# anneouyang/OuterSPACE

Measured on AMD Instinct MI355X. Metric: spgemm_output_nnz_per_s, higher is better.
Workload: dtype f64

## Files before the change

outerspace_amd/csrc/osp_kernels.h:

```cpp
#pragma once
#include <type_traits>
#include "osp_prims.h"

namespace osp {

template <class T> struct TileCap;
#ifndef OSP_TILE_CAP_F32
#define OSP_TILE_CAP_F32 1792
#endif
template <> struct TileCap<float> { static constexpr int value = OSP_TILE_CAP_F32; };
#ifndef OSP_TILE_CAP_F64
#define OSP_TILE_CAP_F64 1536
#endif
template <> struct TileCap<double> { static constexpr int value = OSP_TILE_CAP_F64; };
constexpr int kMergeThreads = 256;
constexpr int kTileMaxRows = kMergeThreads - 1;
constexpr int kMulThreads = 256;
#ifndef OSP_MUL_PER_WAVE
#define OSP_MUL_PER_WAVE 2048
#endif
constexpr int kMulPerWave = OSP_MUL_PER_WAVE;
constexpr int kMulPerBlock = kMulPerWave * (kMulThreads / kWave);
#ifndef OSP_MUL_BATCH_MAX
#define OSP_MUL_BATCH_MAX 4096
// ... 1005 lines not shown
                d.rcnt = vrun_end[rb - 1] - d.rbeg;
            }
        }
    }
    desc[pos] = d;
}
__global__ void chain_rows_kernel(const uint32_t *heavy_rows, uint32_t nlong, const uint32_t *tile_rows0, uint32_t ntiles0,
                                  const uint64_t *vbase, const uint32_t *tile_rows1, uint32_t ntiles1, uint32_t *j0,
                                  uint32_t *tb, uint32_t *cntm1) {
    const uint32_t h = blockIdx.x * blockDim.x + threadIdx.x;
    if (h > nlong) return;
    if (h == nlong) { tb[h] = ntiles1; return; }
    j0[h] = (uint32_t)lower_bound_dev(tile_rows0, 0, (uint64_t)ntiles0, heavy_rows[h]);
    const uint32_t b = (uint32_t)lower_bound_dev(tile_rows1, 0, (uint64_t)ntiles1, vbase[h]);
    const uint32_t e = (uint32_t)lower_bound_dev(tile_rows1, 0, (uint64_t)ntiles1, vbase[h + 1]);
    tb[h] = b;
    cntm1[h] = e - b - 1;
}
__global__ void chain_finish_kernel(const uint32_t *heavy_rows, uint32_t nlong, const uint64_t *vbase, const int64_t *vptr,
                                    const uint64_t *out_end, uint64_t r_end, int64_t *c_rowptr) {
    const uint32_t h = blockIdx.x * blockDim.x + threadIdx.x;
    if (h < nlong) c_rowptr[heavy_rows[h]] = vptr[vbase[h]];
    if (h == 0) c_rowptr[r_end] = (int64_t)*out_end;
}

#ifdef OSP_CHECK_DESC
__device__ unsigned long long osp_desc_bad[16];
#define OSP_DESC_CHECK(t_, d_) do { if ((t_) < ntiles) { const TileDesc g_ = desc[(t_)]; \
    if (g_.s != (d_).s || g_.n != (d_).n || g_.ra != (d_).ra || g_.nr != (d_).nr || g_.lvl != (d_).lvl) { \
        if (atomicAdd(&osp_desc_bad[0], 1ull) == 0) { osp_desc_bad[1] = (t_); osp_desc_bad[2] = tid; osp_desc_bad[3] = (d_).s; osp_desc_bad[4] = g_.s; \
            osp_desc_bad[5] = (d_).n; osp_desc_bad[6] = g_.n; osp_desc_bad[7] = (d_).lvl; osp_desc_bad[8] = blockIdx.x; osp_desc_bad[9] = NT; } \
        (d_) = g_; } } } while (0)
__device__ unsigned long long *osp_crumbs;
#define OSP_CRUMB(ph_, a_, b_, c_) do { if (tid == 0 && osp_crumbs) { volatile unsigned long long *p_ = osp_crumbs + (size_t)(blockIdx.x & 4095u) * 8u; \
    p_[1] = t; p_[2] = d.s; p_[3] = d.n; p_[4] = (a_); p_[5] = (b_); p_[6] = (c_); p_[7] = d.ra; \
    p_[0] = (unsigned long long)(ph_) | ((unsigned long long)NT << 8) | ((unsigned long long)ABL << 32); __threadfence_system(); } } while (0)
#else
#define OSP_DESC_CHECK(t_, d_)
#define OSP_CRUMB(ph_, a_, b_, c_)
#endif

#ifdef OSP_MERGE_PROF
__device__ unsigned long long osp_merge_prof[16];
#define OSP_PROF_DECL __shared__ unsigned long long prof_acc[12]; if (tid < 12) prof_acc[tid] = 0; __syncthreads(); unsigned long long prof_t = clock64();
#define OSP_PROF_MARK(k) do { if (tid == 0) { const unsigned long long now_ = clock64(); prof_acc[k] += now_ - prof_t; prof_t = now_; } } while (0)
#define OSP_PROF_FLUSH do { if (tid == 0) for (int k_ = 0; k_ < 12; k_++) atomicAdd(&osp_merge_prof[k_], prof_acc[k_]); } while (0)
#else
#define OSP_PROF_DECL
#define OSP_PROF_MARK(k)
#define OSP_PROF_FLUSH
#endif

constexpr int kMergeMaxWgs = 5;
template <class T, int NT, int CAP, int MAXWG = kMergeMaxWgs, int ABL = 0>
constexpr int merge_wgs_per_cu() {
    const int wgs = (160 * 1024) / (int)(sizeof(MergeSmem<T, NT, CAP>) + ((ABL & 64) ? CAP * sizeof(T) : 0) + 64);
    return wgs > MAXWG ? MAXWG : wgs;
}
template <class T, int NT, int CAP, int MAXWG = kMergeMaxWgs, int ABL = 0>
constexpr int merge_waves_per_simd() {
    const int w = (merge_wgs_per_cu<T, NT, CAP, MAXWG, ABL>() * NT + 255) / 256;
    return w > 8 ? 8 : (w < 1 ? 1 : w);
}
template <class T, int NT, int ABL = 0, int CAP = TileCap<T>::value, int MAXWG = kMergeMaxWgs, bool RA = (OSP_RANK_ATOMIC != 0), bool GA = false>
__global__ __launch_bounds__(NT, (merge_waves_per_simd<T, NT, CAP, MAXWG, ABL>())) void merge_tiles_kernel(
    const TileDesc *__restrict__ desc, uint32_t ntiles, const MergeLevels<T> lvl, int colbits, uint64_t *tile_status,
    uint32_t *ticket, const uint64_t *__restrict__ out_base_p, uint32_t *__restrict__ c_col, T *__restrict__ c_val,
    uint64_t *__restrict__ out_end_p, const ChunkTable<T> ct = ChunkTable<T>{}, uint32_t nshards = 1, uint32_t *abort_word = nullptr,
    const GatherArgs<T> ga = GatherArgs<T>{}) {
    __shared__ MergeSmem<T, NT, CAP> sm;
    __shared__ TileDesc s_dnext;
    __shared__ uint32_t s_tnext;
    constexpr bool ROWWISE = (ABL & 64) != 0;
    __shared__ T rwval[ROWWISE ? CAP : 1];
    constexpr int kTileCap = CAP;
    constexpr int NW = NT / kWave;
    constexpr int LPT = (kTileCap + NT - 1) / NT;
    constexpr int ITERS = (kTileCap / NW + kWave - 1) / kWave;
    constexpr int IPT = LPT;
    constexpr int DPT = (kDigits + NT - 1) / NT;
    static_assert(kTileMaxRows + 1 <= NT, "row offsets are fetched one per thread");
    unsigned tid = threadIdx.x, lane = lane_id(), w = tid >> 6;
    uint32_t shard = 0;
    if constexpr (GA) { if (tid < (uint32_t)kTileCap / 32u) sm.gbits[tid] = 0; }
    if (tid == 0) {
        if (nshards > 1) shard = atomicAdd(&ticket[nshards * kTicketStride], 1u) % nshards;
        const uint32_t t0 = (ABL & 4) ? blockIdx.x : take_ticket(ticket, nshards, shard, ntiles);
        s_tnext = t0;
        if (t0 < ntiles) s_dnext = desc[t0];
    }
    __syncthreads();
#ifndef OSP_TEST_NO_LATE_GUARD
    if (s_tnext >= ntiles) return;
#endif
    const uint64_t out_base = (ABL & 32) ? 0ull : *out_base_p;
    const uint32_t colmask = colbits < 32 ? ((1u << colbits) - 1u) : 0xffffffffu;
    uint32_t t = s_tnext;
    TileDesc d = s_dnext;
    OSP_CRUMB(5, ntiles, d.lvl, d.nr);
    uint64_t ro = 0;
    PartWords<T> lrec[LPT];
    constexpr uint32_t kSpan = (uint32_t)kTileCap / NW;
    static_assert(!GA || (kTileCap % (NW * kWave) == 0 && (int)kSpan == LPT * kWave), "gathered tiles: a wave's span is LPT wave-loads");
    uint32_t ix0 = GA ? w * kSpan + lane : tid;
    constexpr uint32_t ixs = GA ? (uint32_t)kWave : (uint32_t)NT;
    auto request = [&](const TileDesc &dd, bool ok) {
        bool fetch = ok && dd.n <= (uint32_t)kTileCap;
        ro = 0;
#ifndef OSP_TEST_NO_LATE_GUARD
        const uint32_t lv_i = dd.lvl & 1u;
#else
        const uint32_t lv_i = dd.lvl;
#endif
        const Part<T> *__restrict__ stage = lvl.stage[lv_i];
        if (fetch && tid <= dd.nr) ro = lvl.row_off[lv_i][dd.ra + tid];
        if (ROWWISE && dd.lvl == 0) fetch = false;
        if constexpr (GA) {
            if (fetch && dd.rcnt != 0) {
                typedef uint32_t u32x2 __attribute__((ext_vector_type(2)));
                const RunDesc<T> *__restrict__ gruns = dd.lvl ? ga.runs : ga.runs0;
                const u32x2 ds2 = *reinterpret_cast<const u32x2 *>(&gruns[tid < dd.rcnt ? dd.rbeg + tid : dd.rbeg]);
                const u32x2 ds3 = *reinterpret_cast<const u32x2 *>(&gruns[tid + NT < dd.rcnt ? dd.rbeg + tid + NT : dd.rbeg]);
                lrec[0].w[0] = ds2.x;
                lrec[0].w[1] = ds2.y;
                lrec[1].w[0] = ds3.x;
                lrec[1].w[1] = ds3.y;
                return;
            }
        }
#pragma unroll
        for (int q = 0; q < LPT; q++) {
            const uint32_t i = ix0 + q * ixs;
            const Part<T> *src = (fetch && i < dd.n) ? &stage[dd.s + i] : reinterpret_cast<const Part<T> *>(desc);
            lrec[q] = load_part_words(src);
        }
    };
    request(d, t < ntiles);
    __syncthreads();
    OSP_PROF_DECL
    while (t < ntiles) {
        if constexpr (GA) { asm volatile("" : "+v"(tid)); lane = tid & 63u; w = tid >> 6; ix0 = w * kSpan + lane; }
        OSP_DESC_CHECK(t, d);
        OSP_CRUMB(1, ntiles, d.lvl, d.nr);
        const uint64_t ra = d.ra, s = d.s, base = lvl.base[d.lvl];
        const uint32_t nr = d.nr, n = d.n;
        int64_t *__restrict__ c_rowptr = lvl.c_rowptr[d.lvl];
        const bool long_row = n > (uint32_t)kTileCap;
        uint32_t tn_reg = ntiles;
        if (long_row) {
            if (w == 0) {
                const uint64_t total = lvl.heavy_nnz[d.lvl][ra];
                const uint64_t excl = (ABL & 2) ? (uint64_t)t * kTileCap : lookback_prefix(tile_status, t, total, abort_word);
                if (lane == 0) {
                    tn_reg = (ABL & 4) ? t + gridDim.x : take_ticket(ticket, nshards, shard, ntiles);
                    c_rowptr[ra] = (int64_t)(out_base + excl);
                    if (t + 1 == ntiles) *out_end_p = out_base + excl + total;
                    s_tnext = tn_reg;
                    if (tn_reg < ntiles) s_dnext = desc[tn_reg];
                }
            }
            __syncthreads();
            t = s_tnext;
            d = s_dnext;
            request(d, t < ntiles);
            __syncthreads();
            continue;
        }
        int rowbits = 0;
        while ((1u << rowbits) < nr) rowbits++;
        const bool relkey = d.kbits != 0;
        const uint32_t cbase = d.cbase;
        const int keybits = relkey ? (int)d.kbits : colbits + rowbits;
        const int nbits = (n && !(ABL & 1)) ? keybits : 0;
        constexpr uint32_t HS = MergeSmem<T, NT, CAP>::kHashWords;
        typedef MergeSmem<T, NT, CAP> Smem;
        static_assert(!OSP_HASH_IN_CNT || offsetof(Smem, cnt) + sizeof(sm.cnt) == offsetof(Smem, pos0) + 4u * HS,
                      "hash table: from pos0 through the digit counters without a gap");
        uint32_t *htab = sm.htab();
        constexpr bool INPLACE = (ABL & 32) != 0;
        const bool early = nbits > 0 && keybits < 32 && !(ABL & 2) && !(ABL & 8) && !INPLACE;
        const bool gath = GA && d.rcnt != 0;
        uint32_t kq[LPT];
        T vq[LPT];
        uint32_t rq[(LPT + 1) / 2];
        constexpr bool kRunInPad = GA && Smem::kWide;
        constexpr bool kKeepPos = GA && Smem::kWide;
        uint32_t bpos[LPT];
        constexpr uint32_t GW = GA ? (uint32_t)kTileCap : 0u;
        constexpr uint32_t HSG = HS - GW;
        uint32_t *gsrc = htab, *htab_g = htab + GW;
        if constexpr (GA) {
            if (gath) {
                static_assert(HS > 2 * GW, "gathered tiles: the run table leaves a hash table of more than two words per entry... of half the entries");
                const uint32_t R = d.rcnt, tile0 = (uint32_t)(s + base);
                const RunDesc<T> *__restrict__ gruns = d.lvl ? ga.runs : ga.runs0;
                for (uint32_t x = tid; x < R; x += NT) {
                    uint32_t dst = lrec[0].w[0], src = lrec[0].w[1];
                    if (x == tid + NT) { dst = lrec[1].w[0]; src = lrec[1].w[1]; }
                    else if (x != tid) { const RunDesc<T> rd = gruns[d.rbeg + x]; dst = rd.dst; src = rd.src; }
                    const uint32_t st = dst - tile0;
                    gsrc[x] = src - st;
                    atomicOr(&sm.gbits[st >> 5], 1u << (st & 31u));
                }
                if (early) {
                    typedef uint32_t u32x4 __attribute__((ext_vector_type(4)));
                    static_assert((offsetof(Smem, pos0) + 4u * GW) % 16 == 0, "gathered tiles: the hash table starts 16-byte aligned");
                    constexpr uint32_t nvec = HSG / 4, tail = HSG % 4;
                    u32x4 *hv = reinterpret_cast<u32x4 *>(htab_g);
                    const u32x4 ones = {0xffffffffu, 0xffffffffu, 0xffffffffu, 0xffffffffu};
                    for (uint32_t i = tid; i < nvec; i += NT) hv[i] = ones;
                    if (tid < tail) htab_g[nvec * 4 + tid] = 0xffffffffu;
                    if (tid == 0) sm.hcount = 0;
                }
            }
        }
        if (!gath && early) {
            if constexpr (ABL & 256) {
                for (uint32_t i = tid; i < HS; i += NT) htab[i] = 0xffffffffu;
            } else {
                static_assert((kTileCap * 4) % 8 == 0, "hash table: 16-byte groups behind an 8-byte aligned start (odd words at both ends singly)");
                typedef uint32_t u32x4 __attribute__((ext_vector_type(4)));
                constexpr uint32_t lead = ((kTileCap * 4) % 16) / 4;
                constexpr uint32_t nvec = (HS - lead) / 4, tail = (HS - lead) % 4;
                u32x4 *hv = reinterpret_cast<u32x4 *>(htab + lead);
                const u32x4 ones = {0xffffffffu, 0xffffffffu, 0xffffffffu, 0xffffffffu};
                for (uint32_t i = tid; i < nvec; i += NT) hv[i] = ones;
                if (tid < lead) htab[tid] = 0xffffffffu;
                if (tid < tail) htab[lead + nvec * 4 + tid] = 0xffffffffu;
            }
            if (tid == 0) sm.hcount = 0;
        }
        if (tid <= nr) sm.rowo[tid] = (uint32_t)(ro - base - s);
        __syncthreads();
        OSP_PROF_MARK(0);
        uint32_t fresh = 0;
        const bool rw_tile = ROWWISE && d.lvl == 0;
        if constexpr (GA) {
            if (gath) {
                uint32_t cnt0 = 0;
                {
                    const uint32_t nwords = w * (kSpan / 32u);
                    static_assert((NW - 1) * (kSpan / 32u) <= (uint32_t)kWave, "gathered tiles: the bits before a wave's span, one word per lane");
                    cnt0 = wave_reduce_sum<uint32_t>(lane < nwords ? (uint32_t)__popc(sm.gbits[lane]) : 0u);
                    cnt0 = (uint32_t)__builtin_amdgcn_readfirstlane((int)cnt0);
                }
#pragma unroll
                for (int q = 0; q < (LPT + 1) / 2; q++) rq[q] = 0;
#pragma unroll
                for (int q = 0; q < LPT; q++) {
                    const uint32_t i = ix0 + q * ixs;
                    const uint32_t wi = w * (kSpan / 32u) + 2u * (uint32_t)q;
                    const uint32_t mlo = sm.gbits[wi], mhi = sm.gbits[wi + 1];
                    const uint32_t below = __builtin_amdgcn_mbcnt_hi(mhi, __builtin_amdgcn_mbcnt_lo(mlo, 0u));
                    const uint32_t own = ((lane < 32 ? mlo >> lane : mhi >> (lane - 32)) & 1u);
                    const uint32_t r = cnt0 + below + own - 1u;
                    cnt0 += (uint32_t)__popc(mlo) + (uint32_t)__popc(mhi);
                    bpos[q] = i < n ? gsrc[r] + i : 0u;
                    rq[q >> 1] |= (i < n ? r : 0u) << (16 * (q & 1));
                }
                uint32_t bc[LPT];
#pragma unroll
                for (int q = 0; q < LPT; q++) bc[q] = ga.b_colidx[bpos[q]];
#pragma unroll
                for (int q = 0; q < LPT; q++) {
                    const uint32_t i = ix0 + q * ixs;
                    if (relkey) {
                        kq[q] = bc[q] - cbase;
                    } else {
                        uint32_t lo = 0, hi = nr;
                        while (hi - lo > 1) { const uint32_t mid = (lo + hi) >> 1; if (sm.rowo[mid] <= i) lo = mid; else hi = mid; }
                        kq[q] = (colbits < 32 ? (lo << colbits) : 0u) | bc[q];
                    }
                    if (i < n) sm.key0[i] = kq[q];
                }
                OSP_PROF_MARK(11);
                if (early) {
                    uint32_t hq[LPT], oq[LPT];
#pragma unroll
                    for (int q = 0; q < LPT; q++) {
                        hq[q] = (uint32_t)(((uint64_t)(kq[q] * 2654435761u) * HSG) >> 32);
                        oq[q] = kq[q];
                        if (ix0 + q * ixs < n) oq[q] = atomicCAS(&htab_g[hq[q]], 0xffffffffu, kq[q]);
                    }
#pragma unroll
                    for (int q = 0; q < LPT; q++) {
                        if (ix0 + q * ixs < n) {
                            uint32_t old = oq[q], h = hq[q];
                            while (old != 0xffffffffu && old != kq[q]) {
                                h = (h + 1 == HSG) ? 0u : h + 1;
                                old = atomicCAS(&htab_g[h], 0xffffffffu, kq[q]);
                            }
                            fresh += old == 0xffffffffu;
                        }
                    }
                }
            }
        }
        if (gath) {
        } else if (rw_tile) {
            if constexpr (ROWWISE) {
                constexpr uint32_t kRwGroup = 16, kRwSteps = 4, kRwUnroll = 4;
                const uint32_t c0 = ct.rowfirst[ra], c1 = ct.rowfirst[ra + nr];
                for (uint32_t cb = c0 + w * kRwGroup; cb < c1; cb += NW * kRwGroup) {
                    const uint32_t c = cb + lane;
                    const bool cv = lane < kRwGroup && c < c1;
                    const uint64_t o0 = cv ? ct.off[c] : 0ull, o1 = cv ? ct.off[c + 1] : 0ull;
                    const uint32_t st = cv ? (uint32_t)(o0 - base - s) : n;
                    const uint32_t en = cv ? (uint32_t)(o1 - base - s) : n;
                    const uint32_t bsv = cv ? ct.bs[c] : 0u;
                    const T av = cv ? ct.a_vals[ct.perm[c]] : T(0);
                    uint32_t lrow = 0;
                    {
                        uint32_t lo = 0, hi = nr;
                        while (hi - lo > 1) { const uint32_t mid = (lo + hi) >> 1; if (sm.rowo[mid] <= st) lo = mid; else hi = mid; }
                        lrow = colbits < 32 ? (lo << colbits) : 0u;
                    }
                    const uint32_t nvalid = min(kRwGroup, c1 - cb);
                    const uint32_t gbeg = wave_bcast(st, 0u), gend = wave_bcast(en, nvalid - 1);
                    for (uint32_t ib0 = gbeg; ib0 < gend; ib0 += kRwUnroll * kWave) {
                        uint32_t bcol[kRwUnroll], crow[kRwUnroll];
                        T bval[kRwUnroll], cav[kRwUnroll];
#pragma unroll
                        for (uint32_t u = 0; u < kRwUnroll; u++) {
                            const uint32_t i = ib0 + u * kWave + lane;
                            uint32_t lo = 0, hi = kRwGroup;
#pragma unroll
                            for (uint32_t step = 0; step < kRwSteps; step++) {
                                const uint32_t mid = (lo + hi) >> 1;
                                const uint32_t sv = (uint32_t)__shfl((int)st, (int)mid);
                                if (sv <= i) lo = mid; else hi = mid;
                            }
                            const uint32_t cst = (uint32_t)__shfl((int)st, (int)lo);
                            const uint32_t cbs = (uint32_t)__shfl((int)bsv, (int)lo);
                            crow[u] = (uint32_t)__shfl((int)lrow, (int)lo);
                            cav[u] = __shfl(av, (int)lo);
                            const uint32_t b = i < gend ? cbs + (i - cst) : 0u;
                            bcol[u] = ct.b_colidx[b];
                            bval[u] = ct.b_vals[b];
                        }
#pragma unroll
                        for (uint32_t u = 0; u < kRwUnroll; u++) {
                            const uint32_t i = ib0 + u * kWave + lane;
                            if (i < gend) {
                                const uint32_t key = crow[u] | bcol[u];
                                sm.key0[i] = key;
                                rwval[i] = cav[u] * bval[u];
                                if (early) {
                                    uint32_t h = (uint32_t)(((uint64_t)(key * 2654435761u) * HS) >> 32);
                                    uint32_t old = atomicCAS(&htab[h], 0xffffffffu, key);
                                    while (old != 0xffffffffu && old != key) {
                                        h = (h + 1 == HS) ? 0u : h + 1;
                                        old = atomicCAS(&htab[h], 0xffffffffu, key);
                                    }
                                    fresh += old == 0xffffffffu;
                                }
                            }
                        }
                    }
                }
            }
        } else {
#pragma unroll
            for (int q = 0; q < LPT; q++) {
                const uint32_t i = ix0 + q * ixs;
                kq[q] = 0;
                if (i < n) {
                    if (relkey) {
                        kq[q] = lrec[q].col() - cbase;
                    } else {
                        uint32_t lo = 0, hi = nr;
                        while (hi - lo > 1) { const uint32_t mid = (lo + hi) >> 1; if (sm.rowo[mid] <= i) lo = mid; else hi = mid; }
                        kq[q] = (colbits < 32 ? (lo << colbits) : 0u) | lrec[q].col();
                    }
                    sm.key0[i] = kq[q];
                }
            }
            if (early) {
                uint32_t hq[LPT], oq[LPT];
#pragma unroll
                for (int q = 0; q < LPT; q++) {
                    hq[q] = (uint32_t)(((uint64_t)(kq[q] * 2654435761u) * HS) >> 32);
                    oq[q] = kq[q];
                    if (ix0 + q * ixs < n) oq[q] = atomicCAS(&htab[hq[q]], 0xffffffffu, kq[q]);
                }
#pragma unroll
                for (int q = 0; q < LPT; q++) {
                    if (ix0 + q * ixs < n) {
                        uint32_t old = oq[q], h = hq[q];
                        while (old != 0xffffffffu && old != kq[q]) {
                            h = (h + 1 == HS) ? 0u : h + 1;
                            old = atomicCAS(&htab[h], 0xffffffffu, kq[q]);
                        }
                        fresh += old == 0xffffffffu;
                    }
                }
            }
        }
        if (early) {
            const uint32_t wsum = wave_incl_scan(fresh);
            if (lane == kWave - 1 && wsum) atomicAdd(&sm.hcount, wsum);
        }
        const uint32_t per = (n + NW - 1) / NW;
        const uint32_t wbeg = min(w * per, n), wend = min(wbeg + per, n);
        int cur = 0;
        __syncthreads();
        if constexpr (GA) {
            if (gath) {
                if (tid < (uint32_t)kTileCap / 32u) sm.gbits[tid] = 0;
                if constexpr (kRunInPad) {
#pragma unroll
                    for (int q = 0; q < LPT; q++) {
                        const uint32_t i = ix0 + q * ixs;
                        if (i < n) sm.pad[i] = (uint16_t)(rq[q >> 1] >> (16 * (q & 1)));
                    }
                }
            }
        }
        OSP_PROF_MARK(1);
        if (early && tid == 0) lookback_publish(tile_status, t, sm.hcount);
        OSP_PROF_MARK(2);
        const int npass = (nbits + kDigitBits - 1) / kDigitBits;
        const int pbits = npass ? (nbits + npass - 1) / npass : 0;
        const uint32_t dmask = (1u << pbits) - 1u;
        const int ndig = 1 << pbits;
        for (int pass = 0, shift = 0; pass < npass; pass++, shift += pbits) {
            uint32_t *ksrc = sm.key(cur), *kdst = sm.key(cur ^ 1);
            uint16_t *psrc = sm.pos(cur), *pdst = sm.pos(cur ^ 1);
            if constexpr (ABL & 128) {
                for (int dd = lane; dd < ndig; dd += kWave) sm.cnt[w][dd] = 0;
            } else {
                uint64_t *c64 = reinterpret_cast<uint64_t *>(sm.cnt[w]);
                for (int dd = lane; dd < (ndig + 3) / 4; dd += kWave) c64[dd] = 0ull;
            }
            uint32_t kreg[ITERS], rreg[ITERS];
            auto rank_span = [&](auto bits_tag) {
                constexpr int BITS = decltype(bits_tag)::value;
#pragma unroll
                for (int it = 0; it < ITERS; it++) {
                    const uint32_t i = wbeg + it * kWave + lane;
                    const bool valid = i < wend;
                    kreg[it] = valid ? ksrc[i] : 0u;
                    const unsigned dg = (kreg[it] >> shift) & dmask;
                    unsigned rk, cntd;
                    wave_match_digit<BITS>(dg, valid, rk, cntd);
                    rreg[it] = 0;
                    if (valid) {
                        const uint32_t c = sm.cnt[w][dg];
                        rreg[it] = c + rk;
                        if (rk == 0) sm.cnt[w][dg] = (uint16_t)(c + cntd);
                    }
                }
            };
            if constexpr (RA) {
            {
                uint32_t(*cnt32)[kDigits / 2] = reinterpret_cast<uint32_t(*)[kDigits / 2]>(sm.cnt);
#pragma unroll
                for (int it = 0; it < ITERS; it++) {
                    const uint32_t i = wbeg + it * kWave + lane;
                    const bool valid = i < wend;
                    kreg[it] = valid ? ksrc[i] : 0u;
                    const unsigned dg = (kreg[it] >> shift) & dmask;
                    const unsigned half = 16u * (dg & 1u);
                    rreg[it] = 0;
                    if (valid) rreg[it] = (atomicAdd(&cnt32[w][dg >> 1], 1u << half) >> half) & 0xffffu;
                }
                (void)rank_span;
            }
            } else {
            if (pbits > kDigitBits - 1) rank_span(std::integral_constant<int, kDigitBits>{});
            else rank_span(std::integral_constant<int, kDigitBits - 1>{});
            }
            __syncthreads();
            OSP_PROF_MARK(3);
            if constexpr ((ABL & 128) != 0 || DPT != 4) {
                const int dpt = (ndig + NT - 1) / NT;
                uint32_t c[DPT][NW], ssum = 0;
#pragma unroll
                for (int q = 0; q < DPT; q++) {
                    const int dg = tid * dpt + q;
                    const bool on = q < dpt && dg < ndig;
#pragma unroll
                    for (int ww = 0; ww < NW; ww++) { c[q][ww] = on ? sm.cnt[ww][dg] : 0u; ssum += c[q][ww]; }
                }
                uint32_t total;
                uint32_t ex = block_excl_scan<uint32_t, NT, false>(ssum, sm.scratch, &total)  ;
#pragma unroll
                for (int q = 0; q < DPT; q++) {
                    const int dg = tid * dpt + q;
                    if (q < dpt && dg < ndig) {
#pragma unroll
                        for (int ww = 0; ww < NW; ww++) { sm.cnt[ww][dg] = (uint16_t)ex; ex += c[q][ww]; }
                    }
                }
            } else {
                const bool on = (int)tid * 4 < ndig;
                uint64_t pk[NW];
                uint32_t ssum = 0;
#pragma unroll
                for (int ww = 0; ww < NW; ww++) {
                    pk[ww] = on ? reinterpret_cast<const uint64_t *>(sm.cnt[ww])[tid] : 0ull;
                    ssum += (uint32_t)(pk[ww] & 0xffffu) + (uint32_t)((pk[ww] >> 16) & 0xffffu) + (uint32_t)((pk[ww] >> 32) & 0xffffu) +
                            (uint32_t)(pk[ww] >> 48);
                }
                uint32_t total;
                uint32_t ex = block_excl_scan<uint32_t, NT, false>(ssum, sm.scratch, &total)  ;
                if (on) {
                    uint32_t o[4][NW];
#pragma unroll
                    for (int q = 0; q < 4; q++) {
#pragma unroll
                        for (int ww = 0; ww < NW; ww++) { o[q][ww] = ex; ex += (uint32_t)(pk[ww] >> (16 * q)) & 0xffffu; }
                    }
#pragma unroll
                    for (int ww = 0; ww < NW; ww++)
                        reinterpret_cast<uint64_t *>(sm.cnt[ww])[tid] = (uint64_t)(o[0][ww] & 0xffffu) | ((uint64_t)(o[1][ww] & 0xffffu) << 16) |
                                                                        ((uint64_t)(o[2][ww] & 0xffffu) << 32) | ((uint64_t)(o[3][ww] & 0xffffu) << 48);
                }
            }
            __syncthreads();
            OSP_PROF_MARK(4);
#pragma unroll
            for (int it = 0; it < ITERS; it++) {
                const uint32_t i = wbeg + it * kWave + lane;
                if (i < wend) {
                    const uint32_t k = kreg[it];
                    const uint32_t dst = (uint32_t)sm.cnt[w][(k >> shift) & dmask] + rreg[it];
                    kdst[dst] = k;
                    pdst[dst] = pass == 0 ? (uint16_t)i : psrc[i];
                }
            }
            cur ^= 1;
            __syncthreads();
            OSP_PROF_MARK(5);
        }
        uint32_t *skey = sm.key(cur);
        uint16_t *spos = sm.pos(cur);
        T *sval = rw_tile ? rwval : sm.vals(cur);
        if (npass == 0) {
            for (uint32_t i = tid; i < n; i += NT) spos[i] = (uint16_t)i;
        }
        OSP_CRUMB(2, npass, cur, nbits);
        if (!rw_tile && !gath) {
            const Part<T> *__restrict__ stg = lvl.stage[d.lvl];
#pragma unroll
            for (int q = 0; q < LPT; q++) {
                const uint32_t i = ix0 + q * ixs;
                vq[q] = load_part_words(i < n ? &stg[s + i] : reinterpret_cast<const Part<T> *>(desc)).val();
            }
        }
        if constexpr (GA) {
            if (gath) {
                const uint32_t tile0 = (uint32_t)(s + base);
                const RunDesc<T> *__restrict__ gruns = d.lvl ? ga.runs : ga.runs0;
                T bv[LPT];
                if constexpr (kKeepPos) {
                    T av[LPT];
#pragma unroll
                    for (int q = 0; q < LPT; q++) {
                        const uint32_t i = ix0 + q * ixs;
                        bv[q] = ga.b_vals[bpos[q]];
                        av[q] = gruns[d.rbeg + (i < n ? (uint32_t)sm.pad[i] : 0u)].av;
                    }
#pragma unroll
                    for (int q = 0; q < LPT; q++) vq[q] = av[q] * bv[q];
                    (void)tile0;
                } else {
                RunDesc<T> rdq[LPT];
#pragma unroll
                for (int q = 0; q < LPT; q++) {
                    const uint32_t i = ix0 + q * ixs;
                    uint32_t r;
                    if constexpr (kRunInPad) r = i < n ? (uint32_t)sm.pad[i] : 0u;
                    else r = (rq[q >> 1] >> (16 * (q & 1))) & 0xffffu;
                    rdq[q] = gruns[d.rbeg + r];
                }
#pragma unroll
                for (int q = 0; q < LPT; q++) {
                    const uint32_t i = ix0 + q * ixs;
                    bv[q] = ga.b_vals[i < n ? rdq[q].src - (rdq[q].dst - tile0) + i : 0u];
                }
#pragma unroll
                for (int q = 0; q < LPT; q++) vq[q] = rdq[q].av * bv[q];
                }
            }
        }
        if (npass == 0) __syncthreads();
        const uint32_t ib = tid * IPT;
        uint32_t heads = 0, hmask = 0;
#pragma unroll
        for (int q = 0; q < IPT; q++) {
            const uint32_t i = ib + q;
            if (i < n) {
                const bool h = (i == 0) || (skey[i] != skey[i - 1]);
                hmask |= (h ? 1u : 0u) << q;
                heads += h;
            }
        }
        if constexpr (kRunInPad) {
            if (gath) __syncthreads();
        }
        if (!rw_tile) {
#pragma unroll
            for (int q = 0; q < LPT; q++) {
                const uint32_t i = ix0 + q * ixs;
                if (i < n) sval[i] = vq[q];
            }
        }
        if (tid == 0) sm.nlongrun = 0;
        uint32_t total;
        uint32_t ex = block_excl_scan<uint32_t, NT, false>(heads, sm.scratch, &total);
        OSP_PROF_MARK(6);
        if (w == 0) {
            const uint64_t excl = INPLACE   ? 0ull
                                 : (ABL & 2) ? (uint64_t)t * kTileCap
                                 : early     ? lookback_prefix<false>(tile_status, t, total, abort_word)
                                             : lookback_prefix<true>(tile_status, t, total, abort_word);
            if (lane == 0) {
                sm.excl = excl;
                tn_reg = (ABL & 4) ? t + gridDim.x : take_ticket(ticket, nshards, shard, ntiles);
            }
        }
        OSP_PROF_MARK(7);
        const uint32_t oslot0 = ex;
#pragma unroll
        for (int q = 0; q < IPT; q++) {
            const uint32_t i = ib + q;
            if (i < n) {
                sm.rank[i] = (uint16_t)ex;
                ex += (hmask >> q) & 1u;
            }
        }
        if (tid == 0) sm.rank[n] = (uint16_t)total;
        static_assert(IPT <= kRunShort, "the part of a run inside one thread's entries is never longer than a head's own share");
        T acc[IPT];
        uint32_t ocol[IPT], lmask = 0, tmask = 0;
        {
            T v[IPT];
#pragma unroll
            for (int q = 0; q < IPT; q++) {
                const uint32_t i = ib + q;
                v[q] = i < n ? sval[spos[i]] : T(0);
            }
            T cur = T(0);
#pragma unroll
            for (int q = 0; q < IPT; q++) {
                const uint32_t i = ib + q;
                const bool hd = (hmask >> q) & 1u;
                cur = hd ? v[q] : cur + v[q];
                const bool nexthd = q + 1 < IPT ? ((hmask >> (q + 1)) & 1u) != 0 : true;
                const bool tail = i < n && (i + 1 >= n || nexthd) && (hmask & ((2u << q) - 1u)) != 0;
                acc[q] = cur;
                ocol[q] = 0;
                tmask |= (tail ? 1u : 0u) << q;
            }
        }
        if (tmask) {
            const int qt = 31 - __builtin_clz(tmask);
            const uint32_t it = ib + (uint32_t)qt;
            if (qt == IPT - 1 && it + 1 < n) {
                const uint32_t ih = ib + (uint32_t)(31 - __builtin_clz(hmask));
                const uint32_t k = skey[it];
                T a = acc[IPT - 1];
                const uint32_t ulim = min(n, ih + (uint32_t)kRunShort);
                uint32_t u = it + 1;
                for (; u < ulim && skey[u] == k; u++) a += sval[spos[u]];
                if (u == ulim && u < n && skey[u] == k) {
                    const uint32_t idx = atomicAdd(&sm.nlongrun, 1u);
                    sm.long_sum()[idx] = a;
                    sm.long_pos()[idx] = (uint16_t)u;
                    lmask |= 1u << (IPT - 1);
                    a = index_as_value<T>(idx);
                }
                acc[IPT - 1] = a;
            }
#pragma unroll
            for (int q = 0; q < IPT; q++) {
                if ((tmask >> q) & 1u) {
                    const uint32_t k = skey[ib + q];
                    ocol[q] = relkey ? k + cbase : (k & colmask);
                }
            }
        }
        if (tid == 0) s_tnext = tn_reg;
        __syncthreads();
        if (const uint32_t nlr = sm.nlongrun) {
            T *lsum = sm.long_sum();
            const uint16_t *lpos = sm.long_pos();
            for (uint32_t r = w; r < nlr; r += NW) {
                const uint32_t u1 = lpos[r], k = skey[u1];
                T a = lsum[r];
                for (uint32_t u0 = u1;; u0 += kWave) {
                    const uint32_t u = u0 + lane;
                    const bool in = u < n && skey[u] == k;
                    const T v = in ? sval[spos[u]] : T(0);
                    const uint64_t m = __ballot(in);
                    const uint32_t c = m == ~0ull ? (uint32_t)kWave : (uint32_t)__builtin_ctzll(~m);
                    for (uint32_t x = 0; x < c; x++) a += wave_bcast(v, x);
                    if (c < (uint32_t)kWave) break;
                }
                if (lane == 0) lsum[r] = a;
            }
            __syncthreads();
        }
        OSP_PROF_MARK(8);
#pragma unroll
        for (int q = 0; q < IPT; q++) {
            if ((tmask >> q) & 1u) {
                const uint32_t slot = oslot0 + (uint32_t)__popc(hmask & ((2u << q) - 1u)) - 1u;
                skey[slot] = ocol[q];
                sval[slot] = ((lmask >> q) & 1u) ? sm.long_sum()[value_as_index<T>(acc[q])] : acc[q];
            }
        }
        if (tid == 0 && tn_reg < ntiles) s_dnext = desc[tn_reg];
        __syncthreads();
        OSP_PROF_MARK(9);
        const uint32_t tn = s_tnext;
        const TileDesc dn = s_dnext;
        OSP_CRUMB(3, total, tn, dn.s);
        request(dn, tn < ntiles);
        if constexpr (INPLACE) {
            Part<T> *outp = const_cast<Part<T> *>(lvl.stage[d.lvl]) + s;
            for (uint32_t o = tid; o < total; o += NT) outp[o] = Part<T>{skey[o], sval[o]};
            if (tid == 0) const_cast<uint32_t *>(lvl.heavy_nnz[d.lvl])[ra] = total;
        } else {
            const uint64_t obase = out_base + sm.excl;
            for (uint32_t o = tid; o < total; o += NT) {
                __builtin_nontemporal_store(skey[o], &c_col[obase + o]);
                __builtin_nontemporal_store(sval[o], &c_val[obase + o]);
            }
            if (tid < nr) c_rowptr[ra + tid] = (int64_t)(obase + sm.rank[sm.rowo[tid]]);
            if (t + 1 == ntiles && tid == 0) *out_end_p = obase + total;
        }
        OSP_CRUMB(4, total, tn, 0);
        t = tn;
        d = dn;
        __syncthreads();
        OSP_PROF_MARK(10);
    }
    OSP_CRUMB(7, ntiles, 0, 0);
    OSP_PROF_FLUSH;
}

constexpr int kBigTileCap = 4096;
constexpr int kBigTileThreads = 512;
struct SegHugeFlag {
    const uint32_t *list;
    const uint64_t *row_off;
    uint32_t cap;
    __device__ uint32_t operator()(uint64_t t) const {
        const uint32_t v = list[t];
        return (row_off[v + 1] - row_off[v]) > (uint64_t)cap ? 1u : 0u;
    }
};
__global__ void seg_partition_kernel(SegHugeFlag f, const uint32_t *scan, uint32_t n, uint32_t *huge, uint32_t *mid) {
    const uint32_t t = blockIdx.x * blockDim.x + threadIdx.x;
    if (t >= n) return;
    if (f(t)) huge[scan[t]] = f.list[t]; else mid[t - scan[t]] = f.list[t];
}
__global__ void seg_tile_desc_kernel(const uint32_t *mid, uint32_t nmid, const uint64_t *vrow_off, const uint32_t *vcol0,
                                     const uint32_t *vcol1, TileDesc *desc) {
    const uint32_t t = blockIdx.x * blockDim.x + threadIdx.x;
    if (t >= nmid) return;
    const uint32_t v = mid[t];
    TileDesc d;
    d.s = vrow_off[v];
    d.ra = v;
    d.nr = 1;
    d.n = (uint32_t)(vrow_off[v + 1] - vrow_off[v]);
    d.lvl = 1;
    d.cbase = vcol0[v];
    const uint64_t range = (uint64_t)(vcol1[v] - vcol0[v]);
    int kb = 1;
    while (kb < 32 && (1ull << kb) < range) kb++;
    d.kbits = (uint32_t)kb;
    d.rbeg = 0;
    d.rcnt = 0;
    desc[t] = d;
}

struct HeavyLen {
    const uint32_t *rows;
    const uint64_t *row_off;
    __device__ uint64_t operator()(uint64_t h) const { return row_off[rows[h] + 1] - row_off[rows[h]]; }
};
__global__ void heavy_fill_kernel(const uint32_t *rows, const uint64_t *hoff, uint32_t nheavy,
                                  const uint64_t *row_off, uint64_t base, int colbits,
                                  const char *stage, uint32_t rec_bytes, uint64_t nh, uint64_t *key, uint32_t *pos) {
    uint64_t x = (uint64_t)blockIdx.x * blockDim.x + threadIdx.x;
    if (x >= nh) return;
    uint64_t h = upper_bound_dev(hoff, 0, (uint64_t)nheavy + 1, x) - 1;
// ... 233 lines not shown
```

outerspace_amd/csrc/osp_pipeline.h:

```cpp
#pragma once

#define OSP_WITH_RA(ctx_, ...)                                               \
    do {                                                                     \
        if ((ctx_)->rank_atomic) { constexpr bool RA = true; __VA_ARGS__; }  \
        else { constexpr bool RA = false; __VA_ARGS__; }                     \
    } while (0)

template <class T> struct Producer {
    virtual ~Producer() {}
    virtual void produce(uint64_t r0, uint64_t r1, bool whole, uint64_t base, uint64_t count,
                         Part<T> *stage, PhaseTimer &tm, const uint32_t *cells = nullptr, Part<T> *qstage = nullptr,
                         const HubArgs *hub = nullptr, bool compact = false, bool has_long = true, bool desc_only = false, bool walk_all = false) = 0;
};

template <class T> struct MergeIO {
    Part<T> *stage;
    const uint64_t *row_off; uint64_t r0, r1, base;
    int64_t *c_rowptr; uint32_t *c_col; T *c_val;
    const uint64_t *out_in; uint64_t *out_out;
    ChunkTable<T> ct{};
    uint32_t *abort_word = nullptr;
    const RunDesc<T> *runs0 = nullptr; const uint32_t *rowfirst0 = nullptr; const uint32_t *b_colidx = nullptr; const T *b_vals = nullptr;
};
template <class T> struct ShortRuns {
// ... 462 lines not shown
        tile_desc_kernel<(int)kCap><<<grid_for(p1.ntiles, 256), 256, 0, s>>>(p1.tile_rows, p1.ntiles, nvirt, vrow_off, 0, 1u, j0, extra,
                                                                           nlong, tb, pl.vcol0, pl.vcol1, desc, pl.ga.runs ? pl.vrun_off : nullptr,
                                                                           pl.vrun_end);
        dbg_sync(s, "tile chain");
    } else {
        desc = sc.get<TileDesc>(ntot);
        tile_desc_kernel<(int)kCap><<<grid_for(p0.ntiles, 256), 256, 0, s>>>(p0.tile_rows, p0.ntiles, r1, io.row_off, base, 0u, nullptr,
                                                                           nullptr, 0u, nullptr, nullptr, nullptr, desc, nullptr, nullptr, io.rowfirst0);
    }
    uint64_t *tile_status = sc.get<uint64_t>(ntot);
    const uint32_t nshards = 1u;
    uint32_t *ticket = sc.get<uint32_t>((uint64_t)(nshards + 1) * kTicketStride);
    zero_async(s, {{tile_status, (uint64_t)ntot * sizeof(uint64_t)}, {ticket, (uint64_t)(nshards + 1) * kTicketStride * sizeof(uint32_t)}});
    dbg_sync(s, "tile planning, splits, over-long segments");
    tm.begin(PH_MERGE_K);
    if (io.ct.enabled) {
        const uint32_t rw_grid = ctx->cus * (uint32_t)merge_wgs_per_cu<T, kMergeThreads, TileCap<T>::value, kMergeMaxWgs, 64>();
        OSP_WITH_RA(ctx, merge_tiles_kernel<T, kMergeThreads, 64, TileCap<T>::value, kMergeMaxWgs, RA>
                    <<<std::min<uint32_t>(ntot, rw_grid), kMergeThreads, 0, s>>>(desc, ntot, lv, colbits, tile_status, ticket, io.out_in, io.c_col,
                                                                                 io.c_val, io.out_out, io.ct, nshards, io.abort_word));
    } else if (pl.ga.runs || io.runs0) {
        GatherArgs<T> ga = pl.ga;
        ga.runs0 = io.runs0;
        if (io.runs0) { ga.b_colidx = io.b_colidx; ga.b_vals = io.b_vals; }
        const uint32_t merge_grid = ctx->cus * (uint32_t)merge_wgs_per_cu<T, kMergeThreads, TileCap<T>::value>();
        OSP_WITH_RA(ctx, merge_tiles_kernel<T, kMergeThreads, 0, TileCap<T>::value, kMergeMaxWgs, RA, true>
                    <<<std::min<uint32_t>(ntot, merge_grid), kMergeThreads, 0, s>>>(desc, ntot, lv, colbits, tile_status, ticket, io.out_in, io.c_col,
                                                                                    io.c_val, io.out_out, ChunkTable<T>{}, nshards, io.abort_word, ga));
    } else {
        const uint32_t merge_grid = ctx->cus * (uint32_t)merge_wgs_per_cu<T, kMergeThreads, TileCap<T>::value>();
        OSP_WITH_RA(ctx, merge_tiles_kernel<T, kMergeThreads, 0, TileCap<T>::value, kMergeMaxWgs, RA>
                    <<<std::min<uint32_t>(ntot, merge_grid), kMergeThreads, 0, s>>>(desc, ntot, lv, colbits, tile_status, ticket, io.out_in, io.c_col,
                                                                                    io.c_val, io.out_out, ChunkTable<T>{}, nshards, io.abort_word));
    }
    tm.end(PH_MERGE_K);
    dbg_sync(s, "merge tiles");
#ifdef OSP_MERGE_PROF
    if (getenv("OSP_VERBOSE")) {
        std::vector<TileDesc> hd(ntot);
        copy_d2h(hd.data(), desc, (size_t)ntot * sizeof(TileDesc), s);
        uint64_t byp[5] = {0}, ent[5] = {0}, gt = 0, ge = 0, gr = 0, bits[33] = {0};
        for (const TileDesc &t : hd) {
            if (t.n > kCap) continue;
            int rb = 0; while ((1u << rb) < t.nr) rb++;
            const int kb = t.kbits ? (int)t.kbits : colbits + rb;
            const int np = std::min(4, (kb + kDigitBits - 1) / kDigitBits);
            byp[np]++; ent[np] += t.n; bits[std::min(kb, 32)] += 1;
            if (t.rcnt) { gt++; ge += t.n; gr += t.rcnt; }
        }
        fprintf(stderr, "[osp]   tiles by sort passes:");
        for (int k = 0; k < 5; k++) if (byp[k]) fprintf(stderr, " %d passes: %llu tiles, %.0f entries each;", k, (unsigned long long)byp[k], (double)ent[k] / byp[k]);
        fprintf(stderr, " gathered: %llu tiles, %.0f entries and %.1f runs each\n[osp]   tiles by key bits:", (unsigned long long)gt, gt ? (double)ge / gt : 0.0, gt ? (double)gr / gt : 0.0);
        for (int k = 0; k <= 32; k++) if (bits[k]) fprintf(stderr, " %d: %llu;", k, (unsigned long long)bits[k]);
        fprintf(stderr, "\n");
    }
    if (getenv("OSP_VERBOSE")) {
        unsigned long long hp[16] = {0}, z[16] = {0};
        OSP_HIP(hipStreamSynchronize(s));
        (void)hipMemcpyFromSymbol(hp, HIP_SYMBOL(osp_merge_prof), sizeof(hp));
        (void)hipMemcpyToSymbol(HIP_SYMBOL(osp_merge_prof), z, sizeof(z));
        static const char *names[12] = {"run table / hash init", "keys + hash count", "publish", "rank", "digit scan", "scatter", "values + heads + scan",
                                        "look-back + ticket", "run sums", "compaction", "output + next tile's request", "gathered: lookup + columns"};
        double tot = 0;
        for (int k = 0; k < 12; k++) tot += (double)hp[k];
        fprintf(stderr, "[osp]   merge kernel, %u tiles, cycles of thread 0 per phase:", ntot);
        for (int k = 0; k < 12; k++) fprintf(stderr, " %s %.1f %%;", names[k], 100.0 * hp[k] / tot);
        fprintf(stderr, " %.0f cycles per tile and workgroup\n", tot / std::max(1u, ntot));
    }
#endif
    res->info.merge_launches++;
    if (p1.nlong) {
        heavy_copy_kernel<T><<<grid_for(p1.nlong, 8), 256, 0, s>>>(p1.long_rows, p1.nlong, seg_src, seg_nnz, vptr, qstage, nullptr, nullptr,
                                                                   io.c_col, io.c_val);
        heavy_copy_rest_kernel<T><<<p1.nlong, 256, 0, s>>>(p1.long_rows, p1.nlong, seg_src, seg_nnz, vptr, qstage, nullptr, nullptr,
                                                           io.c_col, io.c_val);
    }
    chain_finish_kernel<<<grid_for(std::max<uint32_t>(p0.nlong, 1), 256), 256, 0, s>>>(p0.long_rows, p0.nlong, vbase, vptr, io.out_out, r1,
                                                                                       io.c_rowptr);
    dbg_sync(s, "copy of reduced segments, chain finish");
    OSP_HIP(hipGetLastError());
}

struct PanelSink {
    osp_panel_fn fn;
    void *user;
};

constexpr uint64_t kPartialsOnDevice = ~0ull;
template <class T>
static void merge_pipeline(Context *ctx, Result *res, Producer<T> &prod, uint64_t M_all, uint64_t N,
                           const uint64_t *d_row_off,
                           uint64_t P, uint64_t cap_cfg, PhaseTimer &tm, uint64_t r_lo = 0, uint64_t r_hi = ~0ull,
                           uint64_t off_lo = 0, const PanelSink *sink = nullptr, const ChunkTable<T> *ct = nullptr,
                           const DirectSrc *ds = nullptr, const std::vector<uint64_t> *cuts = nullptr, const ShortRuns<T> *sr = nullptr) {
    if (r_hi == ~0ull) r_hi = M_all;
    const uint64_t M = r_hi - r_lo;
    res->info.M = M;
    res->info.row_begin = r_lo;
    res->info.row_end = r_hi;
    hipStream_t s = ctx->stream;
    Scratch sc(ctx);
    const int colbits = std::max(1, bits_for(N));

    const uint64_t E = 4 + sizeof(T);
    uint64_t cap_c;
    uint64_t *ub = sc.get<uint64_t>(M + 1);
// ... 324 lines not shown
```

Baseline: 65.56 billion.

## Specialise merge tile body by per-tile round count to skip empty slots

The merge kernel now picks one of up to three compile-time instantiations of its tile body based on how many per-thread rounds a tile actually needs (ceil(n/NT)), rather than always iterating LPT slots. Loads, hashing, radix ranking, value gathers and segmented scans run only Q rounds for small tiles, and each wave's span and per-wave share change to match. This is meant to cut wasted work and register pressure on partially filled tiles. In exchange, code size roughly triples for the body, and the per-wave partitioning of keys changes, which could affect correctness or occupancy.

Result: faster. 67.11 billion, median of 6 (+2.4%).

```diff
diff --git a/outerspace_amd/csrc/osp_kernels.h b/outerspace_amd/csrc/osp_kernels.h
--- a/outerspace_amd/csrc/osp_kernels.h
+++ b/outerspace_amd/csrc/osp_kernels.h
@@ -1081,6 +1081,12 @@
 #endif
 
 constexpr int kMergeMaxWgs = 5;
+#ifndef OSP_TILE_ROUNDS
+#define OSP_TILE_ROUNDS 3
+#endif
+constexpr int kTileRoundClasses = OSP_TILE_ROUNDS > 1 ? OSP_TILE_ROUNDS : 1;
+static_assert(kTileRoundClasses <= 3, "OSP_TILE_ROUNDS: at most three bodies");
+constexpr int tile_class_rounds(int lpt, int c, int K) { return (lpt * c + K - 1) / K; }
 template <class T, int NT, int CAP, int MAXWG = kMergeMaxWgs, int ABL = 0>
 constexpr int merge_wgs_per_cu() {
     const int wgs = (160 * 1024) / (int)(sizeof(MergeSmem<T, NT, CAP>) + ((ABL & 64) ? CAP * sizeof(T) : 0) + 64);
@@ -1106,7 +1112,6 @@
     constexpr int NW = NT / kWave;
     constexpr int LPT = (kTileCap + NT - 1) / NT;
     constexpr int ITERS = (kTileCap / NW + kWave - 1) / kWave;
-    constexpr int IPT = LPT;
     constexpr int DPT = (kDigits + NT - 1) / NT;
     static_assert(kTileMaxRows + 1 <= NT, "row offsets are fetched one per thread");
     unsigned tid = threadIdx.x, lane = lane_id(), w = tid >> 6;
@@ -1129,12 +1134,20 @@
     OSP_CRUMB(5, ntiles, d.lvl, d.nr);
     uint64_t ro = 0;
     PartWords<T> lrec[LPT];
-    constexpr uint32_t kSpan = (uint32_t)kTileCap / NW;
-    static_assert(!GA || (kTileCap % (NW * kWave) == 0 && (int)kSpan == LPT * kWave), "gathered tiles: a wave's span is LPT wave-loads");
-    uint32_t ix0 = GA ? w * kSpan + lane : tid;
+    static_assert(!GA || kTileCap % (NW * kWave) == 0, "gathered tiles: a wave's span is a whole number of wave-loads");
+    static_assert(ITERS <= LPT, "sort passes: a wave's share of a full tile in LPT wave-loads");
+    constexpr int K = kTileRoundClasses;
+    constexpr int Q1 = tile_class_rounds(LPT, 1, K), Q2 = tile_class_rounds(LPT, K > 1 ? 2 : 1, K);
+    auto tile_rounds = [&](uint32_t n_) -> uint32_t {
+        const uint32_t qn = (uint32_t)__builtin_amdgcn_readfirstlane((int)((n_ + NT - 1) / NT));
+        return K > 1 && qn <= (uint32_t)Q1 ? (uint32_t)Q1 : K > 2 && qn <= (uint32_t)Q2 ? (uint32_t)Q2 : (uint32_t)LPT;
+    };
+    uint32_t ix0 = tid;
     constexpr uint32_t ixs = GA ? (uint32_t)kWave : (uint32_t)NT;
     auto request = [&](const TileDesc &dd, bool ok) {
         bool fetch = ok && dd.n <= (uint32_t)kTileCap;
+        const uint32_t qr = tile_rounds(dd.n);
+        const uint32_t rx0 = GA ? w * (uint32_t)kWave * qr + lane : tid;
         ro = 0;
 #ifndef OSP_TEST_NO_LATE_GUARD
         const uint32_t lv_i = dd.lvl & 1u;
@@ -1159,7 +1172,8 @@
         }
 #pragma unroll
         for (int q = 0; q < LPT; q++) {
-            const uint32_t i = ix0 + q * ixs;
+            if ((K > 1 && q >= Q1 && qr <= (uint32_t)Q1) || (K > 2 && q >= Q2 && qr <= (uint32_t)Q2)) continue;
+            const uint32_t i = rx0 + q * ixs;
             const Part<T> *src = (fetch && i < dd.n) ? &stage[dd.s + i] : reinterpret_cast<const Part<T> *>(desc);
             lrec[q] = load_part_words(src);
         }
@@ -1168,7 +1182,7 @@
     __syncthreads();
     OSP_PROF_DECL
     while (t < ntiles) {
-        if constexpr (GA) { asm volatile("" : "+v"(tid)); lane = tid & 63u; w = tid >> 6; ix0 = w * kSpan + lane; }
+        if constexpr (GA || K > 1) { asm volatile("" : "+v"(tid)); lane = tid & 63u; w = tid >> 6; }
         OSP_DESC_CHECK(t, d);
         OSP_CRUMB(1, ntiles, d.lvl, d.nr);
         const uint64_t ra = d.ra, s = d.s, base = lvl.base[d.lvl];
@@ -1195,6 +1209,11 @@
             __syncthreads();
             continue;
         }
+        auto tile_body = [&](auto rounds_tag) __attribute__((always_inline)) {
+        constexpr int Q = decltype(rounds_tag)::value;
+        static_assert(Q >= 1 && Q <= LPT, "rounds of a tile body");
+        constexpr int SQ = K > 1 ? Q : ITERS;
+        ix0 = GA ? w * (uint32_t)(kWave * Q) + lane : tid;
         int rowbits = 0;
         while ((1u << rowbits) < nr) rowbits++;
         const bool relkey = d.kbits != 0;
@@ -1268,17 +1287,17 @@
             if (gath) {
                 uint32_t cnt0 = 0;
                 {
-                    const uint32_t nwords = w * (kSpan / 32u);
-                    static_assert((NW - 1) * (kSpan / 32u) <= (uint32_t)kWave, "gathered tiles: the bits before a wave's span, one word per lane");
+                    const uint32_t nwords = w * (2u * Q);
+                    static_assert((NW - 1) * 2 * LPT <= kWave, "gathered tiles: the bits before a wave's span, one word per lane");
                     cnt0 = wave_reduce_sum<uint32_t>(lane < nwords ? (uint32_t)__popc(sm.gbits[lane]) : 0u);
                     cnt0 = (uint32_t)__builtin_amdgcn_readfirstlane((int)cnt0);
                 }
 #pragma unroll
                 for (int q = 0; q < (LPT + 1) / 2; q++) rq[q] = 0;
 #pragma unroll
-                for (int q = 0; q < LPT; q++) {
+                for (int q = 0; q < Q; q++) {
                     const uint32_t i = ix0 + q * ixs;
-                    const uint32_t wi = w * (kSpan / 32u) + 2u * (uint32_t)q;
+                    const uint32_t wi = w * (2u * Q) + 2u * (uint32_t)q;
                     const uint32_t mlo = sm.gbits[wi], mhi = sm.gbits[wi + 1];
                     const uint32_t below = __builtin_amdgcn_mbcnt_hi(mhi, __builtin_amdgcn_mbcnt_lo(mlo, 0u));
                     const uint32_t own = ((lane < 32 ? mlo >> lane : mhi >> (lane - 32)) & 1u);
@@ -1289,9 +1308,9 @@
                 }
                 uint32_t bc[LPT];
 #pragma unroll
-                for (int q = 0; q < LPT; q++) bc[q] = ga.b_colidx[bpos[q]];
-#pragma unroll
-                for (int q = 0; q < LPT; q++) {
+                for (int q = 0; q < Q; q++) bc[q] = ga.b_colidx[bpos[q]];
+#pragma unroll
+                for (int q = 0; q < Q; q++) {
                     const uint32_t i = ix0 + q * ixs;
                     if (relkey) {
                         kq[q] = bc[q] - cbase;
@@ -1306,13 +1325,13 @@
                 if (early) {
                     uint32_t hq[LPT], oq[LPT];
 #pragma unroll
-                    for (int q = 0; q < LPT; q++) {
+                    for (int q = 0; q < Q; q++) {
                         hq[q] = (uint32_t)(((uint64_t)(kq[q] * 2654435761u) * HSG) >> 32);
                         oq[q] = kq[q];
                         if (ix0 + q * ixs < n) oq[q] = atomicCAS(&htab_g[hq[q]], 0xffffffffu, kq[q]);
                     }
 #pragma unroll
-                    for (int q = 0; q < LPT; q++) {
+                    for (int q = 0; q < Q; q++) {
                         if (ix0 + q * ixs < n) {
                             uint32_t old = oq[q], h = hq[q];
                             while (old != 0xffffffffu && old != kq[q]) {
@@ -1390,7 +1409,7 @@
             }
         } else {
 #pragma unroll
-            for (int q = 0; q < LPT; q++) {
+            for (int q = 0; q < Q; q++) {
                 const uint32_t i = ix0 + q * ixs;
                 kq[q] = 0;
                 if (i < n) {
@@ -1407,13 +1426,13 @@
             if (early) {
                 uint32_t hq[LPT], oq[LPT];
 #pragma unroll
-                for (int q = 0; q < LPT; q++) {
+                for (int q = 0; q < Q; q++) {
                     hq[q] = (uint32_t)(((uint64_t)(kq[q] * 2654435761u) * HS) >> 32);
                     oq[q] = kq[q];
                     if (ix0 + q * ixs < n) oq[q] = atomicCAS(&htab[hq[q]], 0xffffffffu, kq[q]);
                 }
 #pragma unroll
-                for (int q = 0; q < LPT; q++) {
+                for (int q = 0; q < Q; q++) {
                     if (ix0 + q * ixs < n) {
                         uint32_t old = oq[q], h = hq[q];
                         while (old != 0xffffffffu && old != kq[q]) {
@@ -1429,7 +1448,7 @@
             const uint32_t wsum = wave_incl_scan(fresh);
             if (lane == kWave - 1 && wsum) atomicAdd(&sm.hcount, wsum);
         }
-        const uint32_t per = (n + NW - 1) / NW;
+        const uint32_t per = K > 1 ? (uint32_t)(kWave * Q) : (n + NW - 1) / NW;
         const uint32_t wbeg = min(w * per, n), wend = min(wbeg + per, n);
         int cur = 0;
         __syncthreads();
@@ -1438,7 +1457,7 @@
                 if (tid < (uint32_t)kTileCap / 32u) sm.gbits[tid] = 0;
                 if constexpr (kRunInPad) {
 #pragma unroll
-                    for (int q = 0; q < LPT; q++) {
+                    for (int q = 0; q < Q; q++) {
                         const uint32_t i = ix0 + q * ixs;
                         if (i < n) sm.pad[i] = (uint16_t)(rq[q >> 1] >> (16 * (q & 1)));
                     }
@@ -1461,11 +1480,11 @@
                 uint64_t *c64 = reinterpret_cast<uint64_t *>(sm.cnt[w]);
                 for (int dd = lane; dd < (ndig + 3) / 4; dd += kWave) c64[dd] = 0ull;
             }
-            uint32_t kreg[ITERS], rreg[ITERS];
+            uint32_t kreg[SQ], rreg[SQ];
             auto rank_span = [&](auto bits_tag) {
                 constexpr int BITS = decltype(bits_tag)::value;
 #pragma unroll
-                for (int it = 0; it < ITERS; it++) {
+                for (int it = 0; it < SQ; it++) {
                     const uint32_t i = wbeg + it * kWave + lane;
                     const bool valid = i < wend;
                     kreg[it] = valid ? ksrc[i] : 0u;
@@ -1484,7 +1503,7 @@
             {
                 uint32_t(*cnt32)[kDigits / 2] = reinterpret_cast<uint32_t(*)[kDigits / 2]>(sm.cnt);
 #pragma unroll
-                for (int it = 0; it < ITERS; it++) {
+                for (int it = 0; it < SQ; it++) {
                     const uint32_t i = wbeg + it * kWave + lane;
                     const bool valid = i < wend;
                     kreg[it] = valid ? ksrc[i] : 0u;
@@ -1549,7 +1568,7 @@
             __syncthreads();
             OSP_PROF_MARK(4);
 #pragma unroll
-            for (int it = 0; it < ITERS; it++) {
+            for (int it = 0; it < SQ; it++) {
                 const uint32_t i = wbeg + it * kWave + lane;
                 if (i < wend) {
                     const uint32_t k = kreg[it];
@@ -1572,7 +1591,7 @@
         if (!rw_tile && !gath) {
             const Part<T> *__restrict__ stg = lvl.stage[d.lvl];
 #pragma unroll
-            for (int q = 0; q < LPT; q++) {
+            for (int q = 0; q < Q; q++) {
                 const uint32_t i = ix0 + q * ixs;
                 vq[q] = load_part_words(i < n ? &stg[s + i] : reinterpret_cast<const Part<T> *>(desc)).val();
             }
@@ -1585,18 +1604,18 @@
                 if constexpr (kKeepPos) {
                     T av[LPT];
 #pragma unroll
-                    for (int q = 0; q < LPT; q++) {
+                    for (int q = 0; q < Q; q++) {
                         const uint32_t i = ix0 + q * ixs;
                         bv[q] = ga.b_vals[bpos[q]];
                         av[q] = gruns[d.rbeg + (i < n ? (uint32_t)sm.pad[i] : 0u)].av;
                     }
 #pragma unroll
-                    for (int q = 0; q < LPT; q++) vq[q] = av[q] * bv[q];
+                    for (int q = 0; q < Q; q++) vq[q] = av[q] * bv[q];
                     (void)tile0;
                 } else {
                 RunDesc<T> rdq[LPT];
 #pragma unroll
-                for (int q = 0; q < LPT; q++) {
+                for (int q = 0; q < Q; q++) {
                     const uint32_t i = ix0 + q * ixs;
                     uint32_t r;
                     if constexpr (kRunInPad) r = i < n ? (uint32_t)sm.pad[i] : 0u;
@@ -1604,20 +1623,21 @@
                     rdq[q] = gruns[d.rbeg + r];
                 }
 #pragma unroll
-                for (int q = 0; q < LPT; q++) {
+                for (int q = 0; q < Q; q++) {
                     const uint32_t i = ix0 + q * ixs;
                     bv[q] = ga.b_vals[i < n ? rdq[q].src - (rdq[q].dst - tile0) + i : 0u];
                 }
 #pragma unroll
-                for (int q = 0; q < LPT; q++) vq[q] = rdq[q].av * bv[q];
+                for (int q = 0; q < Q; q++) vq[q] = rdq[q].av * bv[q];
                 }
             }
         }
         if (npass == 0) __syncthreads();
+        constexpr int IPT = Q;
         const uint32_t ib = tid * IPT;
         uint32_t heads = 0, hmask = 0;
 #pragma unroll
-        for (int q = 0; q < IPT; q++) {
+        for (int q = 0; q < Q; q++) {
             const uint32_t i = ib + q;
             if (i < n) {
                 const bool h = (i == 0) || (skey[i] != skey[i - 1]);
@@ -1630,7 +1650,7 @@
         }
         if (!rw_tile) {
 #pragma unroll
-            for (int q = 0; q < LPT; q++) {
+            for (int q = 0; q < Q; q++) {
                 const uint32_t i = ix0 + q * ixs;
                 if (i < n) sval[i] = vq[q];
             }
@@ -1652,7 +1672,7 @@
         OSP_PROF_MARK(7);
         const uint32_t oslot0 = ex;
 #pragma unroll
-        for (int q = 0; q < IPT; q++) {
+        for (int q = 0; q < Q; q++) {
             const uint32_t i = ib + q;
             if (i < n) {
                 sm.rank[i] = (uint16_t)ex;
@@ -1666,13 +1686,13 @@
         {
             T v[IPT];
 #pragma unroll
-            for (int q = 0; q < IPT; q++) {
+            for (int q = 0; q < Q; q++) {
                 const uint32_t i = ib + q;
                 v[q] = i < n ? sval[spos[i]] : T(0);
             }
             T cur = T(0);
 #pragma unroll
-            for (int q = 0; q < IPT; q++) {
+            for (int q = 0; q < Q; q++) {
                 const uint32_t i = ib + q;
                 const bool hd = (hmask >> q) & 1u;
                 cur = hd ? v[q] : cur + v[q];
@@ -1703,7 +1723,7 @@
                 acc[IPT - 1] = a;
             }
 #pragma unroll
-            for (int q = 0; q < IPT; q++) {
+            for (int q = 0; q < Q; q++) {
                 if ((tmask >> q) & 1u) {
                     const uint32_t k = skey[ib + q];
                     ocol[q] = relkey ? k + cbase : (k & colmask);
@@ -1733,7 +1753,7 @@
         }
         OSP_PROF_MARK(8);
 #pragma unroll
-        for (int q = 0; q < IPT; q++) {
+        for (int q = 0; q < Q; q++) {
             if ((tmask >> q) & 1u) {
                 const uint32_t slot = oslot0 + (uint32_t)__popc(hmask & ((2u << q) - 1u)) - 1u;
                 skey[slot] = ocol[q];
@@ -1765,6 +1785,10 @@
         d = dn;
         __syncthreads();
         OSP_PROF_MARK(10);
+        };
+        if (const uint32_t rounds = tile_rounds(n); K > 1 && rounds == (uint32_t)Q1) tile_body(std::integral_constant<int, Q1>{});
+        else if (K > 2 && rounds == (uint32_t)Q2) tile_body(std::integral_constant<int, Q2>{});
+        else tile_body(std::integral_constant<int, LPT>{});
     }
     OSP_CRUMB(7, ntiles, 0, 0);
     OSP_PROF_FLUSH;
diff --git a/outerspace_amd/csrc/osp_pipeline.h b/outerspace_amd/csrc/osp_pipeline.h
--- a/outerspace_amd/csrc/osp_pipeline.h
+++ b/outerspace_amd/csrc/osp_pipeline.h
@@ -538,6 +538,19 @@
         for (int k = 0; k < 5; k++) if (byp[k]) fprintf(stderr, " %d passes: %llu tiles, %.0f entries each;", k, (unsigned long long)byp[k], (double)ent[k] / byp[k]);
         fprintf(stderr, " gathered: %llu tiles, %.0f entries and %.1f runs each\n[osp]   tiles by key bits:", (unsigned long long)gt, gt ? (double)ge / gt : 0.0, gt ? (double)gr / gt : 0.0);
         for (int k = 0; k <= 32; k++) if (bits[k]) fprintf(stderr, " %d: %llu;", k, (unsigned long long)bits[k]);
+        constexpr int lpt = ((int)kCap + kMergeThreads - 1) / kMergeThreads;
+        uint64_t byq[lpt + 1] = {0}, slots = 0, need = 0, run = 0;
+        for (const TileDesc &t : hd) {
+            if (t.n > kCap) continue;
+            const int q = std::max(1, (int)((t.n + kMergeThreads - 1) / kMergeThreads));
+            int body = lpt;
+            for (int c = kTileRoundClasses; c >= 1; c--) if (q <= tile_class_rounds(lpt, c, kTileRoundClasses)) body = tile_class_rounds(lpt, c, kTileRoundClasses);
+            byq[q]++; slots += lpt; need += q; run += body;
+        }
+        fprintf(stderr, "\n[osp]   tiles by rounds (Q = ceil(n / %d)):", kMergeThreads);
+        for (int q = 1; q <= lpt; q++) fprintf(stderr, " Q=%d: %llu;", q, (unsigned long long)byq[q]);
+        fprintf(stderr, " slot-rounds needed %.1f %%, run %.1f %% of %d per tile (%d bodies)", slots ? 100.0 * need / slots : 0.0,
+                slots ? 100.0 * run / slots : 0.0, lpt, kTileRoundClasses);
         fprintf(stderr, "\n");
     }
     if (getenv("OSP_VERBOSE")) {
```
